# uni-medical/UniMedVL

Measured on AMD Instinct MI355X. Metric: VQA greedy decode tokens/s, UniMedVL-14B (BAGEL-7B-MoT dims), batch 8 x 448x448 per GPU, higher is better.
Workload: dtype bf16; 1 GPU; configs[1]: UniMedVL-14B bf16 VQA greedy decode, batch=8 448x448, 1xMI355X; batch_per_gpu=8, image=448x448, parallelism=dp1, decode=hipGraph

## Files before the change

### unimedvl_amd/csrc/gemm_skinny.h

```cpp
#pragma once
#include "common.h"
#include "../../include/unimedvl_hip.h"
#include "gemm_epilogue.h"
#include "gemm_internal.h"
#include "quant.h"

#define SK_WAVES 8
#define SK_XMAX 16

template <int NT_>
struct SkBf16 {
    static constexpr int NT = NT_, KH = 1;
    static constexpr bool HALVES = false;
    struct Unit { bf16x8 w[NT]; };
    int TH, tile_elems;
    bool rowlane;
    const bf16_t* wbase[NT];
    __device__ __forceinline__ SkBf16(const umv_gemm_args& a, int KT, int NTT, int, int nt0, int lane) {
        const int r = lane & 15, g = lane >> 4;
        TH = a.tile_rows > 0 ? a.tile_rows : 16;
        tile_elems = 4 * TH * 8;
        rowlane = r < TH;
#pragma unroll
        for (int t = 0; t < NT; ++t) {
            const bool tv = (nt0 + t) < NTT;
            wbase[t] = a.wp + ((int64_t)(tv ? nt0 + t : 0) * KT) * tile_elems + (g * TH + (rowlane ? r : 0)) * 8;
        }
    }
    __device__ __forceinline__ void load(Unit& b, int kt, bool ok) const {
#pragma unroll
        for (int t = 0; t < NT; ++t)
            b.w[t] = (ok && rowlane) ? __builtin_nontemporal_load(reinterpret_cast<const bf16x8*>(wbase[t] + (int64_t)kt * tile_elems)) : zero_frag();
    }
    __device__ __forceinline__ void frags(const Unit& b, bf16x8 (&wf)[KH][NT]) const {
#pragma unroll
        for (int t = 0; t < NT; ++t) wf[0][t] = b.w[t];
    }
};

template <int NT_>
struct SkE4m3 {
    static constexpr int NT = NT_, KH = 2, TH = 16;
    static constexpr bool HALVES = false;
    struct Unit { u32x4 w[NT]; };
    const uint8_t* wbase[NT];
    float wscale[NT];
    __device__ __forceinline__ SkE4m3(const umv_gemm_args& a, int KT8, int NTT, int, int nt0, int lane) {
        const uint8_t* wq = reinterpret_cast<const uint8_t*>(a.wp);
#pragma unroll
        for (int t = 0; t < NT; ++t) {
            const bool tv = (nt0 + t) < NTT;
            const int nt = tv ? nt0 + t : 0;
            wbase[t] = wq + ((int64_t)nt * KT8 * 64 + lane) * 16;
            wscale[t] = a.w_scale[nt * 16 + (lane & 15)];
        }
    }
    __device__ __forceinline__ void load(Unit& b, int kt, bool ok) const {
#pragma unroll
        for (int t = 0; t < NT; ++t)
            b.w[t] = ok ? __builtin_nontemporal_load(reinterpret_cast<const u32x4*>(wbase[t] + (int64_t)kt * 1024)) : (u32x4){0u, 0u, 0u, 0u};
    }
    __device__ __forceinline__ void frags(const Unit& b, bf16x8 (&wf)[KH][NT]) const {
#pragma unroll
        for (int t = 0; t < NT; ++t) cvt_fp8x16(b.w[t], wscale[t], wf[0][t], wf[1][t]);
    }
};

template <int NP>
struct SkMxfp4 {
    static constexpr int NT = 2 * NP, KH = 2, TH = 16;
    static constexpr bool HALVES = false;
    struct Unit { u32x4 w[NP]; uint32_t s[NP]; };
    const uint8_t* wbase[NP];
    const uint8_t* sbase[NP];
    __device__ __forceinline__ SkMxfp4(const umv_gemm_args& a, int KT8, int, int NPT, int, int lane) {
        const uint8_t* img = reinterpret_cast<const uint8_t*>(a.wp);
        const uint8_t* scales = img + (int64_t)NPT * KT8 * 1024;
        const int p0 = blockIdx.x * NP;
#pragma unroll
        for (int i = 0; i < NP; ++i) {
            const int p = (p0 + i) < NPT ? p0 + i : 0;
            wbase[i] = img + ((int64_t)p * KT8 * 64 + lane) * 16;
            sbase[i] = scales + ((int64_t)p * KT8 * 16 + (lane & 15)) * 4;
        }
    }
    __device__ __forceinline__ void load(Unit& b, int kt, bool ok) const {
#pragma unroll
        for (int i = 0; i < NP; ++i) {
            b.w[i] = ok ? __builtin_nontemporal_load(reinterpret_cast<const u32x4*>(wbase[i] + (int64_t)kt * 1024)) : (u32x4){0u, 0u, 0u, 0u};
            b.s[i] = ok ? *reinterpret_cast<const uint32_t*>(sbase[i] + (int64_t)kt * 64) : 0x7F7F7F7Fu;
        }
    }
    __device__ __forceinline__ void frags(const Unit& b, bf16x8 (&wf)[KH][NT]) const {
#pragma unroll
        for (int i = 0; i < NP; ++i) {
            const uint32_t s = b.s[i];
            wf[0][2 * i] = cvt_fp4x8(b.w[i].x, e8m0_scale(s & 0xFFu));
            wf[1][2 * i] = cvt_fp4x8(b.w[i].y, e8m0_scale((s >> 8) & 0xFFu));
            wf[0][2 * i + 1] = cvt_fp4x8(b.w[i].z, e8m0_scale((s >> 16) & 0xFFu));
            wf[1][2 * i + 1] = cvt_fp4x8(b.w[i].w, e8m0_scale(s >> 24));
        }
    }
};

typedef __attribute__((ext_vector_type(2))) unsigned short umv_u16x2;
__device__ __forceinline__ uint32_t z13_pk_mad(uint32_t q, uint32_t mul, uint32_t add) {
    const umv_u16x2 r = __builtin_bit_cast(umv_u16x2, q) * __builtin_bit_cast(umv_u16x2, mul) + __builtin_bit_cast(umv_u16x2, add);
    return __builtin_bit_cast(uint32_t, r);
}
__device__ __forceinline__ uint32_t z13_pk_shr8(uint32_t q) {
    const umv_u16x2 r = __builtin_bit_cast(umv_u16x2, q) >> (umv_u16x2){8, 8};
    return __builtin_bit_cast(uint32_t, r);
}
template <int E>
__device__ __forceinline__ bf16x8 z13_frag(uint32_t sm0, uint32_t sm1, uint32_t n, uint32_t t, uint32_t mul, uint32_t base7, uint32_t emask) {
    constexpr int EA = 2 * E, EB = 2 * E + 1;
    const uint32_t ta = EA < 4 ? t << (4 - EA) : t >> (EA - 4), tb = EB < 4 ? t << (4 - EB) : t >> (EB - 4);
    const uint32_t qa = (ta & 0x10101010u) | (n & 0x0F0F0F0Fu), qb = (tb & 0x10101010u) | ((n >> 4) & 0x0F0F0F0Fu);
    const uint32_t e[4] = {z13_pk_mad(qa, mul, base7), z13_pk_mad(z13_pk_shr8(qa), mul, base7), z13_pk_mad(qb, mul, base7),
                           z13_pk_mad(z13_pk_shr8(qb), mul, base7)};
    const uint32_t p[4] = {__builtin_amdgcn_perm(sm0, sm0, 0x01010000u), __builtin_amdgcn_perm(sm0, sm0, 0x03030202u),
                           __builtin_amdgcn_perm(sm1, sm1, 0x01010000u), __builtin_amdgcn_perm(sm1, sm1, 0x03030202u)};
    u32x4 o;
    o.x = (e[0] & emask) | (p[0] & ~emask);
    o.y = (e[1] & emask) | (p[1] & ~emask);
    o.z = (e[2] & emask) | (p[2] & ~emask);
    o.w = (e[3] & emask) | (p[3] & ~emask);
    return __builtin_bit_cast(bf16x8, o);
}

#define Z13_RECORD 3328
__host__ __device__ __forceinline__ int64_t z13_head_bytes(int NPT) { return ((int64_t)NPT * 16 + 255) / 256 * 256; }

template <int NP>
struct SkZ13 {
    static constexpr int NT = 2 * NP, KH = 2, TH = 16;
    static constexpr bool HALVES = true;
    struct Unit { u32x4 sm[NP][2]; u32x4 n[NP]; uint32_t t[NP]; };
    const uint8_t* rec[NP];
    uint32_t base7[NP];
    uint32_t lane16, lane4;
    __device__ __forceinline__ SkZ13(const umv_gemm_args& a, int KT8, int, int NPT, int, int lane) {
        const uint8_t* img = reinterpret_cast<const uint8_t*>(a.wp);
        const int p0 = blockIdx.x * NP;
#pragma unroll
        for (int i = 0; i < NP; ++i) {
            const int p = (p0 + i) < NPT ? p0 + i : 0;
            rec[i] = img + z13_head_bytes(NPT) + (int64_t)p * KT8 * Z13_RECORD;
            const uint32_t b = reinterpret_cast<const uint32_t*>(img)[4 * p + 2] & 0xFFu;
            base7[i] = (b << 7) * 0x10001u;
        }
        lane16 = (uint32_t)lane * 16u;
        lane4 = 3072u + (uint32_t)lane * 4u;
    }
    __device__ __forceinline__ void load(Unit& b, int kt, bool ok) const {
        const int ktu = __builtin_amdgcn_readfirstlane(kt);
#pragma unroll
        for (int i = 0; i < NP; ++i) {
            const uint8_t* r = rec[i] + (int64_t)ktu * Z13_RECORD;
            const u32x4 z = {0u, 0u, 0u, 0u};
            b.sm[i][0] = ok ? __builtin_nontemporal_load(reinterpret_cast<const u32x4*>(r + lane16)) : z;
            b.sm[i][1] = ok ? __builtin_nontemporal_load(reinterpret_cast<const u32x4*>(r + 1024 + lane16)) : z;
            b.n[i] = ok ? __builtin_nontemporal_load(reinterpret_cast<const u32x4*>(r + 2048 + lane16)) : z;
            b.t[i] = ok ? __builtin_nontemporal_load(reinterpret_cast<const uint32_t*>(r + lane4)) : 0u;
        }
    }
    __device__ __forceinline__ void frags(const Unit& b, bf16x8 (&wf)[KH][NT], bool in0, bool in1) const {
        const bool v0 = __builtin_amdgcn_readfirstlane((int)in0) != 0, v1 = __builtin_amdgcn_readfirstlane((int)in1) != 0;
#pragma unroll
        for (int i = 0; i < NP; ++i) {
            const uint32_t mul0 = v0 ? 0xFF80FF80u : 0u, mul1 = v1 ? 0xFF80FF80u : 0u;
            const uint32_t b0 = v0 ? base7[i] : 0u, b1 = v1 ? base7[i] : 0u;
            const uint32_t m0 = v0 ? 0x7F807F80u : 0xFFFFFFFFu, m1 = v1 ? 0x7F807F80u : 0xFFFFFFFFu;
            wf[0][2 * i] = z13_frag<0>(b.sm[i][0].x, b.sm[i][0].y, b.n[i].x, b.t[i], mul0, b0, m0);
            wf[1][2 * i] = z13_frag<1>(b.sm[i][0].z, b.sm[i][0].w, b.n[i].y, b.t[i], mul1, b1, m1);
            wf[0][2 * i + 1] = z13_frag<2>(b.sm[i][1].x, b.sm[i][1].y, b.n[i].z, b.t[i], mul0, b0, m0);
            wf[1][2 * i + 1] = z13_frag<3>(b.sm[i][1].z, b.sm[i][1].w, b.n[i].w, b.t[i], mul1, b1, m1);
        }
    }
};

template <int NW, int NT, int MB>
__device__ __forceinline__ void skinny16_reduce_epilogue(const umv_gemm_args& a, float* red, const f32x4 (&acc)[NT][MB], int tid,
                                                         int lane, int wave, int nt0, int NTT, int nsplit, int TH) {
    constexpr int E4 = NT * MB;
#pragma unroll
    for (int t = 0; t < NT; ++t)
#pragma unroll
        for (int mb = 0; mb < MB; ++mb) reinterpret_cast<f32x4*>(red)[(wave * E4 + t * MB + mb) * 64 + lane] = acc[t][mb];
    __syncthreads();
    EpiCtx e{a.bias, a.residual, a.ldr, a.out, a.ldo, a.N, a.epilogue};
    if (nsplit > 1) {
        e.out = reinterpret_cast<float*>(a.out) + (int64_t)blockIdx.y * a.split_stride;
        e.flags = UMV_EPI_OUT_F32;
    }
    if (a.epilogue & UMV_EPI_SWIGLU) {
        for (int idx = tid; idx < (NT / 2) * MB * 64; idx += NW * 64) {
            int l = idx & 63;
            int f = idx >> 6;
            int pair = f / MB, mb = f % MB;
            f32x4 sg = {0, 0, 0, 0}, su = {0, 0, 0, 0};
#pragma unroll
            for (int w = 0; w < NW; ++w) {
                sg += reinterpret_cast<f32x4*>(red)[(w * E4 + (2 * pair) * MB + mb) * 64 + l];
                su += reinterpret_cast<f32x4*>(red)[(w * E4 + (2 * pair + 1) * MB + mb) * 64 + l];
            }
            int m = mb * 16 + (l & 15);
            int ntile = nt0 + 2 * pair;
            if (m < a.M && ntile < NTT) {
                int64_t orow = a.row_idx ? (int64_t)a.row_idx[m] : (int64_t)m;
                int c0 = (ntile >> 1) * 16 + (l >> 4) * 4;
                float gg[4] = {sg.x, sg.y, sg.z, sg.w}, uu[4] = {su.x, su.y, su.z, su.w};
                epi_swiglu4(e, orow, c0, a.N / 2, gg, uu);
            }
        }
    } else {
        for (int idx = tid; idx < E4 * 64; idx += NW * 64) {
            int l = idx & 63;
            int f = idx >> 6;
            int t = f / MB, mb = f % MB;
            f32x4 s = {0, 0, 0, 0};
#pragma unroll
            for (int w = 0; w < NW; ++w) s += reinterpret_cast<f32x4*>(red)[(w * E4 + f) * 64 + l];
            int m = mb * 16 + (l & 15);
            int n0 = (nt0 + t) * TH + (l >> 4) * 4;
            int nend = min(a.N, (nt0 + t) * TH + TH);
            const bool valid = m < a.M && n0 < nend;
            float fin[4] = {0.f, 0.f, 0.f, 0.f};
            if (valid) {
                int64_t orow = a.row_idx ? (int64_t)a.row_idx[m] : (int64_t)m;
                EpiCtx et = e;
                et.N = nend;
                epi_store4(et, orow, n0, s.x, s.y, s.z, s.w, fin);
            }
            if (a.argmax_partial && nt0 + t < NTT)
                epi_argmax_tile(a.argmax_partial, NTT, m, nt0 + t, l, valid, n0, nend, fin, a.sample_temperature, a.sample_seed, a.sample_step);
        }
    }
}

template <class F, int MB, int U, int XL>
struct SkBuf {
    typename F::Unit w[U];
    bf16x8 x[U][F::KH][MB];
    u32x4 xp[XL ? U * F::KH / 2 : 1][XL == 1 ? 1 : (XL ? 2 * MB : 1)];
};

template <class F, int MB, int U, bool DB, int NORM, int XL>
__device__ __forceinline__ void gemm_skinny_body(const umv_gemm_args& a, int KT, int NTT, int NPT) {
    constexpr int NT = F::NT, KH = F::KH;
    extern __shared__ __attribute__((aligned(16))) float red[];
    const int tid = threadIdx.x;
    const int lane = tid & 63, wave = tid >> 6;
    const int r = lane & 15, g = lane >> 4;
    const int nt0 = blockIdx.x * NT;

    const bf16_t* xrow[MB];
    bool xvalid[MB];
#pragma unroll
    for (int mb = 0; mb < MB; ++mb) {
        int m = mb * 16 + r;
        xvalid[mb] = m < a.M;
        int64_t row = xvalid[mb] ? (a.row_idx ? (int64_t)a.row_idx[m] : (int64_t)m) : 0;
        xrow[mb] = a.x + row * a.ldx;
    }
    f32x4 acc[NT][MB];
#pragma unroll
    for (int t = 0; t < NT; ++t)
#pragma unroll
        for (int mb = 0; mb < MB; ++mb) acc[t][mb] = (f32x4){0.f, 0.f, 0.f, 0.f};

    const int nsplit = a.k_splits > 1 ? a.k_splits : 1;
    constexpr int SG = F::HALVES ? KH : 1;
    const int KTG = KT * SG;
    const int kts = (KTG + nsplit - 1) / nsplit;
    const int ks0 = (int)blockIdx.y * kts, ks1 = min(KTG, ks0 + kts);
    const int kt_per = (max(0, ks1 - ks0) + SK_WAVES - 1) / SK_WAVES;
    const int g_begin = ks0 + wave * kt_per;
    const int g_end = min(ks1, g_begin + kt_per);
    const int kt_begin = g_begin / SG;
    const int kt_end = g_end > g_begin ? (g_end + SG - 1) / SG : kt_begin;
    constexpr int UPL = 2 / KH;
    const int kt_lo = XL != 0 ? (kt_begin & -UPL) : kt_begin;
    const int nk = max(0, kt_end - kt_lo);
    const int nchunks = (nk + U - 1) / U;
    const F f(a, KT, NTT, NPT, nt0, lane);
    static_assert(!XL || ((U * KH) % 2 == 0 && NORM == 0), "full-line x staging: whole lines per chunk, no fused norm");
    static_assert(!F::HALVES || NORM == 0, "half-unit slices: no fused norm");
    static_assert(XL != 1 || MB == 1, "one-piece staging serves one 16-row tile of at most 8 valid rows");
    constexpr int XLN = U * KH / 2, XLP = XL == 1 ? 1 : 2 * MB;
    const int xchunk = (lane & 7) ^ ((lane >> 3) & 7);
    const bf16_t* xprow[XL ? XLP : 1];
    bool xpvalid[XL ? XLP : 1];
    if constexpr (XL != 0) {
#pragma unroll
        for (int q = 0; q < XLP; ++q) {
            const int m = q * 8 + (lane >> 3);
            xpvalid[q] = m < a.M;
            const int64_t row = xpvalid[q] ? (a.row_idx ? (int64_t)a.row_idx[m] : (int64_t)m) : 0;
            xprow[q] = a.x + row * a.ldx + xchunk * 8;
        }
    }
    char* xstage = reinterpret_cast<char*>(red) + wave * (XLN * XLP * 1024);
    auto load_chunk = [&](int c, SkBuf<F, MB, U, XL>& b) {
        if constexpr (XL != 0) {
#pragma unroll
            for (int ln = 0; ln < XLN; ++ln) {
                const int kt = kt_lo + c * U + ln * UPL;
                const int k = kt * (32 * KH) + xchunk * 8;
#pragma unroll
                for (int q = 0; q < XLP; ++q)
                    b.xp[ln][q] = (kt < kt_end && xpvalid[q] && k < a.K) ? *reinterpret_cast<const u32x4*>(xprow[q] + (int64_t)kt * (32 * KH))
                                                                         : (u32x4){0u, 0u, 0u, 0u};
            }
        }
#pragma unroll
        for (int u = 0; u < U; ++u) {
            const int kt = kt_lo + c * U + u;
            const bool ok = kt >= kt_begin && kt < kt_end;
            f.load(b.w[u], kt, ok);
            if (!NORM && XL == 0) {
#pragma unroll
                for (int h = 0; h < KH; ++h) {
                    const int k = kt * (32 * KH) + h * 32 + g * 8;
#pragma unroll
                    for (int mb = 0; mb < MB; ++mb) b.x[u][h][mb] = (ok && xvalid[mb] && k < a.K) ? ldg_frag(xrow[mb] + k) : zero_frag();
                }
            }
        }
    };
    SkBuf<F, MB, U, XL> b0, b1;
    if (nchunks > 0) load_chunk(0, b0);

    constexpr int MP = NORM ? NORM : 8;
    bf16_t* xl = reinterpret_cast<bf16_t*>(red + SK_WAVES * NT * MB * 4 * 64 + SK_WAVES * 16);
    if constexpr (NORM != 0) {
        static_assert(!NORM || MB == 1, "fused RMSNorm supports M <= 16");
        float* part = red + SK_WAVES * NT * MB * 4 * 64;
        const int rr = tid & (MP - 1);
        constexpr int sh = MP == 8 ? 3 : 4;
        constexpr int XS = MP;
        const int nslots = KT * 4 * MP;
        const bool rowok = rr < a.M;
        const bf16_t* xr = a.x + (rowok ? (a.row_idx ? (int64_t)a.row_idx[rr] : (int64_t)rr) : 0) * a.ldx;
        {
            bf16x8 xv[XS];
#pragma unroll
            for (int i = 0; i < XS; ++i) {
                const int sidx = tid + i * SK_WAVES * 64;
                const int k = (sidx >> (sh + 2)) * 32 + ((sidx >> sh) & 3) * 8;
                xv[i] = (sidx < nslots && k < a.K && rowok) ? ldg_frag(xr + k) : zero_frag();
            }
            float ss = 0.f;
#pragma unroll
            for (int i = 0; i < XS; ++i) {
#pragma unroll
                for (int j = 0; j < 8; ++j) {
                    float fv = bf2f((bf16_t)xv[i][j]);
                    ss += fv * fv;
                }
                const int sidx = tid + i * SK_WAVES * 64;
                if (sidx < nslots) *reinterpret_cast<bf16x8*>(xl + (int64_t)sidx * 8) = xv[i];
            }
            if (MP == 8) ss += __shfl_xor(ss, 8, 64);
            ss += __shfl_xor(ss, 16, 64);
            ss += __shfl_xor(ss, 32, 64);
            if (lane < MP) part[wave * 16 + lane] = ss;
        }
        bf16x8 wv[XS];
#pragma unroll
        for (int i = 0; i < XS; ++i) {
            const int sidx = tid + i * SK_WAVES * 64;
            const int k = (sidx >> (sh + 2)) * 32 + ((sidx >> sh) & 3) * 8;
            wv[i] = (sidx < nslots && k < a.K) ? ldg_frag(a.norm_w + k) : zero_frag();
        }
        __syncthreads();
        float tot = 0.f;
#pragma unroll
        for (int w = 0; w < SK_WAVES; ++w) tot += part[w * 16 + rr];
        const float rstd = rsqrt_ieee(tot / (float)a.K + a.norm_eps);
#pragma unroll
        for (int i = 0; i < XS; ++i) {
            const int sidx = tid + i * SK_WAVES * 64;
            if (sidx < nslots) {
                bf16x8 v = *reinterpret_cast<const bf16x8*>(xl + (int64_t)sidx * 8), o;
#pragma unroll
                for (int j = 0; j < 8; ++j) o[j] = (short)f2bf(bf2f((bf16_t)wv[i][j]) * rbf(bf2f((bf16_t)v[j]) * rstd));
                *reinterpret_cast<bf16x8*>(xl + (int64_t)sidx * 8) = o;
            }
        }
        __syncthreads();
    }
    auto consume = [&](SkBuf<F, MB, U, XL>& b, int c) {
        if constexpr (NORM != 0) {
#pragma unroll
            for (int u = 0; u < U; ++u) {
                const int kt = min(kt_begin + c * U + u, KT - 1);
                bf16x8 xf = *reinterpret_cast<const bf16x8*>(xl + ((int64_t)(kt * 4 + g) * MP + (r & (MP - 1))) * 8);
                bf16x8 wf[KH][NT];
                f.frags(b.w[u], wf);
#pragma unroll
                for (int t = 0; t < NT; ++t) acc[t][0] = mfma16(wf[0][t], xf, acc[t][0]);
            }
        } else {
            if constexpr (XL != 0) {
#pragma unroll
                for (int ln = 0; ln < XLN; ++ln)
#pragma unroll
                    for (int q = 0; q < XLP; ++q) *reinterpret_cast<u32x4*>(xstage + (ln * XLP + q) * 1024 + lane * 16) = b.xp[ln][q];
                const int rr = XL == 1 ? (r & 7) : r;
#pragma unroll
                for (int u = 0; u < U; ++u)
#pragma unroll
                    for (int h = 0; h < KH; ++h)
#pragma unroll
                        for (int mb = 0; mb < MB; ++mb) {
                            const int j = u * KH + h;
                            b.x[u][h][mb] = *reinterpret_cast<const bf16x8*>(xstage + (j >> 1) * (XLP * 1024) + (mb * 16 + rr) * 128 +
                                                                             ((((j & 1) * 4 + g) ^ (rr & 7)) << 4));
                        }
            }
#pragma unroll
            for (int u = 0; u < U; ++u) {
                bf16x8 wf[KH][NT];
                if constexpr (F::HALVES) {
                    const int g0 = (kt_lo + c * U + u) * SG;
                    f.frags(b.w[u], wf, g0 >= g_begin && g0 < g_end, g0 + 1 >= g_begin && g0 + 1 < g_end);
                } else {
                    f.frags(b.w[u], wf);
                }
#pragma unroll
                for (int h = 0; h < KH; ++h)
#pragma unroll
                    for (int t = 0; t < NT; ++t)
#pragma unroll
                        for (int mb = 0; mb < MB; ++mb) acc[t][mb] = mfma16(wf[h][t], b.x[u][h][mb], acc[t][mb]);
            }
        }
    };
    for (int c = 0; c < nchunks; c += 2) {
        if (DB && c + 1 < nchunks) load_chunk(c + 1, b1);
        consume(b0, c);
        if (c + 1 < nchunks) {
            if (!DB) load_chunk(c + 1, b1);
            if (c + 2 < nchunks && DB) load_chunk(c + 2, b0);
            consume(b1, c + 1);
            if (c + 2 < nchunks && !DB) load_chunk(c + 2, b0);
        }
    }
    if constexpr (XL != 0) __syncthreads();
    skinny16_reduce_epilogue<SK_WAVES, NT, MB>(a, red, acc, tid, lane, wave, nt0, NTT, nsplit, f.TH);
}

static int skinny_xl() {
    static const int v = umv_env_int("UMV_SKINNY_XL", 2);
    return v;
}

template <int MB, int NT, int U, int KH, int NORM, class Kernel, class... Args>
static int launch_skinny_body(Kernel kernel, const umv_gemm_args& a, int KT, int NTT, hipStream_t s, Args... args) {
    size_t lds = (size_t)SK_WAVES * NT * MB * 4 * 64 * sizeof(float);
    if (NORM) lds += SK_WAVES * 16 * sizeof(float) + (size_t)KT * 4 * NORM * 16;
    auto go = [&](auto XLV) {
        constexpr int XL = decltype(XLV)::value;
        const void* fn = reinterpret_cast<const void*>(kernel(XLV));
        const size_t xl = (size_t)SK_WAVES * (U * KH / 2) * (XL == 1 ? 1 : 2 * MB) * 1024;
        const size_t bytes = XL != 0 && xl > lds ? xl : lds;
        static bool attr_set[UMV_MAX_DEVICES] = {};
        if (bytes > 64 * 1024 && umv_first_on_device(attr_set)) (void)hipFuncSetAttribute(fn, hipFuncAttributeMaxDynamicSharedMemorySize, (int)bytes);
        umv_gemm_args ka = a;
        void* argv[] = {&ka, &args...};
        (void)hipLaunchKernel(fn, dim3((NTT + NT - 1) / NT, a.k_splits > 1 ? a.k_splits : 1), dim3(SK_WAVES * 64), argv, bytes, s);
        UMV_LAUNCH_CHECK();
        return UMV_OK;
    };
    if constexpr (NORM == 0 && (U * KH) % 2 == 0) {
        const int mode = skinny_xl();
        if (mode && (mode > 1 || a.M > 8) && (a.ldx % 64) == 0 && ((uintptr_t)a.x % 128) == 0) {
            if constexpr (MB == 1) {
                if (a.M <= 8) return go(std::integral_constant<int, 1>{});
            }
            return go(std::integral_constant<int, 2>{});
        }
    }
    return go(std::integral_constant<int, 0>{});
}
```

### unimedvl_amd/csrc/gemm_z13.hip

```cpp
#include "common.h"
#include "../../include/unimedvl_hip.h"
#include "gemm_skinny.h"

template <int MB, int NP, int U, int XL = 0>
__global__ __launch_bounds__(SK_WAVES * 64) void gemm_skinny13_kernel(umv_gemm_args a, const uint8_t* z13, int KT8, int NTT, int NPT) {
    const int KT = 2 * KT8, nsplit = a.k_splits > 1 ? a.k_splits : 1;
    const int kts = (KT + nsplit - 1) / nsplit;
    const int ks0 = (int)blockIdx.y * kts, ks1 = min(KT, ks0 + kts);
    uint64_t any = 0;
    if (ks1 > ks0) {
        const int b0 = ks0 >> 4, b1 = (ks1 + 15) >> 4;
        const uint64_t range = (b1 - b0 >= 64 ? ~0ull : ((1ull << (b1 - b0)) - 1ull)) << b0;
        const uint64_t* flags = reinterpret_cast<const uint64_t*>(z13);
#pragma unroll
        for (int i = 0; i < NP; ++i) {
            const int p = (int)blockIdx.x * NP + i;
            if (p < NPT) any |= flags[2 * p] & range;
        }
    }
    if (any != 0) {
        gemm_skinny_body<SkBf16<2 * NP>, MB, 2 * U, true, 0, XL>(a, KT, NTT, 0);
    } else {
        a.wp = reinterpret_cast<const uint16_t*>(z13);
        gemm_skinny_body<SkZ13<NP>, MB, U, true, 0, XL>(a, KT8, NTT, NPT);
    }
}

template <int MB, int NP, int U>
static int launch_skinny13(const umv_gemm_args& a, const uint8_t* z13, int KT8, int NTT, int NPT, hipStream_t s) {
    return launch_skinny_body<MB, 2 * NP, U, 2, 0>([](auto XL) { return &gemm_skinny13_kernel<MB, NP, U, decltype(XL)::value>; }, a, KT8,
                                                   NTT, s, z13, KT8, NTT, NPT);
}

extern "C" int umv_gemm_z13w(const umv_gemm_args* ap, const void* z13, umv_stream_t stream) {
    UMV_CHECK(ap != nullptr, UMV_ERR_ARG, "gemm_z13w: null args");
    umv_gemm_args a = *ap;
    UMV_CHECK(a.x && a.wp && a.out && z13, UMV_ERR_ARG, "gemm_z13w: null pointer (x, wp = the bf16 image, out and z13 are required)");
    UMV_CHECK(!a.w_scale, UMV_ERR_ARG, "gemm_z13w: w_scale must be NULL");
    if (const int rc = umv_gemm_check_args(a, "gemm_z13w", 32)) return rc;
    UMV_CHECK((a.K % 64) == 0 && a.K <= 32768, UMV_ERR_UNSUPPORTED, "gemm_z13w: K (%d) must be a multiple of 64 and <= 32768", a.K);
    UMV_CHECK(a.M <= 64, UMV_ERR_UNSUPPORTED, "gemm_z13w: the 13-bit image is the decode (M <= 64) layout; use umv_gemm_bf16 for M=%d", a.M);
    UMV_CHECK(!a.norm_w && (a.tile_rows == 0 || a.tile_rows == 16), UMV_ERR_UNSUPPORTED, "gemm_z13w: no fused norm / th-row tiles");
    UMV_CHECK(a.k_splits <= 1 || (!(a.epilogue & UMV_EPI_SWIGLU) && a.split_stride > 0 && a.k_splits <= 64), UMV_ERR_UNSUPPORTED,
              "gemm_z13w: split-K (k_splits=%d) needs no SwiGLU, split_stride > 0, k_splits <= 64", a.k_splits);
    UMV_CHECK(!a.argmax_partial || (a.k_splits <= 1 && !a.row_idx && !(a.epilogue & (UMV_EPI_SWIGLU | UMV_EPI_OUT_F32))), UMV_ERR_UNSUPPORTED,
              "gemm_z13w: argmax_partial needs bf16 out, no SwiGLU / split-K / row_idx");
    UMV_CHECK(a.sample_temperature >= 0.f && (a.sample_temperature == 0.f || a.argmax_partial), UMV_ERR_ARG,
              "gemm_z13w: sample_temperature (%g) is a mode of the argmax_partial epilogue and must be >= 0", (double)a.sample_temperature);
    UMV_CHECK(((uintptr_t)z13 % 256) == 0, UMV_ERR_ARG, "gemm_z13w: the 13-bit image must be 256-byte aligned");
    if (a.M == 0) return UMV_OK;
    hipStream_t s = (hipStream_t)stream;
    const uint8_t* z = reinterpret_cast<const uint8_t*>(z13);
    const int KT8 = a.K / 64, NTT = (a.N + 15) / 16, NPT = (NTT + 1) / 2;
    if (a.k_splits > 1) {
        if (a.M <= 16) return launch_skinny13<1, 2, 1>(a, z, KT8, NTT, NPT, s);
        if (a.M <= 32) return launch_skinny13<2, 2, 1>(a, z, KT8, NTT, NPT, s);
        return launch_skinny13<4, 1, 1>(a, z, KT8, NTT, NPT, s);
    }
    const bool two = (a.epilogue & UMV_EPI_SWIGLU) || NTT >= 1024;
    if (a.M <= 16) return launch_skinny13<1, 1, 2>(a, z, KT8, NTT, NPT, s);
    if (a.M <= 32) return two ? launch_skinny13<2, 2, 1>(a, z, KT8, NTT, NPT, s) : launch_skinny13<2, 1, 2>(a, z, KT8, NTT, NPT, s);
    if (two && !a.argmax_partial && a.K >= 1024) return umv_gemm_bf16(&a, stream);
    return launch_skinny13<4, 1, 1>(a, z, KT8, NTT, NPT, s);
}
```

Measured before the change: 2720 tokens/s.

## Add ring-buffered prefetch pipeline to 13-bit skinny GEMM and overlap flag check

The 13-bit decode GEMM for M<=16 now uses a three-deep ring of load buffers with unrolled steady-state stages, replacing the previous double-buffered loop with U=2. The per-block exception-flag check and base exponent read move into the Z13 body. They now come from a header vector loaded in the constructor, and the check runs after the first chunk's loads are already issued, so the flag lookup no longer serialises ahead of the weight stream. If any row is flagged, the body returns false and the kernel falls back to the bf16 path, which now uses a separately chosen unroll. The deeper ring raises register pressure, and fallback blocks issue some wasted Z13 loads.

```diff
diff --git a/unimedvl_amd/csrc/gemm_skinny.h b/unimedvl_amd/csrc/gemm_skinny.h
--- a/unimedvl_amd/csrc/gemm_skinny.h
+++ b/unimedvl_amd/csrc/gemm_skinny.h
@@ -1,4 +1,5 @@
 #pragma once
+#include <utility>
 #include "common.h"
 #include "../../include/unimedvl_hip.h"
 #include "gemm_epilogue.h"
@@ -10,7 +11,7 @@
 
 template <int NT_>
 struct SkBf16 {
-    static constexpr int NT = NT_, KH = 1;
+    static constexpr int NT = NT_, KH = 1, RING = 0;
     static constexpr bool HALVES = false;
     struct Unit { bf16x8 w[NT]; };
     int TH, tile_elems;
@@ -40,7 +41,7 @@
 
 template <int NT_>
 struct SkE4m3 {
-    static constexpr int NT = NT_, KH = 2, TH = 16;
+    static constexpr int NT = NT_, KH = 2, TH = 16, RING = 0;
     static constexpr bool HALVES = false;
     struct Unit { u32x4 w[NT]; };
     const uint8_t* wbase[NT];
@@ -68,7 +69,7 @@
 
 template <int NP>
 struct SkMxfp4 {
-    static constexpr int NT = 2 * NP, KH = 2, TH = 16;
+    static constexpr int NT = 2 * NP, KH = 2, TH = 16, RING = 0;
     static constexpr bool HALVES = false;
     struct Unit { u32x4 w[NP]; uint32_t s[NP]; };
     const uint8_t* wbase[NP];
@@ -132,26 +133,42 @@
 #define Z13_RECORD 3328
 __host__ __device__ __forceinline__ int64_t z13_head_bytes(int NPT) { return ((int64_t)NPT * 16 + 255) / 256 * 256; }
 
-template <int NP>
+template <int NP, int R>
 struct SkZ13 {
-    static constexpr int NT = 2 * NP, KH = 2, TH = 16;
+    static constexpr int NT = 2 * NP, KH = 2, TH = 16, RING = R;
     static constexpr bool HALVES = true;
     struct Unit { u32x4 sm[NP][2]; u32x4 n[NP]; uint32_t t[NP]; };
     const uint8_t* rec[NP];
+    u32x4 head[NP];
+    int npairs;
     uint32_t base7[NP];
     uint32_t lane16, lane4;
     __device__ __forceinline__ SkZ13(const umv_gemm_args& a, int KT8, int, int NPT, int, int lane) {
         const uint8_t* img = reinterpret_cast<const uint8_t*>(a.wp);
         const int p0 = blockIdx.x * NP;
+        npairs = NPT - p0;
 #pragma unroll
         for (int i = 0; i < NP; ++i) {
             const int p = (p0 + i) < NPT ? p0 + i : 0;
             rec[i] = img + z13_head_bytes(NPT) + (int64_t)p * KT8 * Z13_RECORD;
-            const uint32_t b = reinterpret_cast<const uint32_t*>(img)[4 * p + 2] & 0xFFu;
-            base7[i] = (b << 7) * 0x10001u;
+            head[i] = *reinterpret_cast<const u32x4*>(img + (int64_t)p * 16);
         }
         lane16 = (uint32_t)lane * 16u;
         lane4 = 3072u + (uint32_t)lane * 4u;
+    }
+    __device__ __forceinline__ bool flagged(int g0, int g1) const {
+        if (g1 <= g0) return false;
+        const int b0 = g0 >> 4, b1 = (g1 + 15) >> 4;
+        const uint64_t range = (b1 - b0 >= 64 ? ~0ull : ((1ull << (b1 - b0)) - 1ull)) << b0;
+        uint64_t any = 0;
+#pragma unroll
+        for (int i = 0; i < NP; ++i)
+            if (i < npairs) any |= ((uint64_t)head[i].y << 32 | head[i].x) & range;
+        return any != 0;
+    }
+    __device__ __forceinline__ void resolve() {
+#pragma unroll
+        for (int i = 0; i < NP; ++i) base7[i] = ((head[i].z & 0xFFu) << 7) * 0x10001u;
     }
     __device__ __forceinline__ void load(Unit& b, int kt, bool ok) const {
         const int ktu = __builtin_amdgcn_readfirstlane(kt);
@@ -246,14 +263,18 @@
     u32x4 xp[XL ? U * F::KH / 2 : 1][XL == 1 ? 1 : (XL ? 2 * MB : 1)];
 };
 
+template <class Fn, int... S>
+__device__ __forceinline__ void sk_each(Fn&& fn, std::integer_sequence<int, S...>) { (fn(std::integral_constant<int, S>{}), ...); }
+
 template <class F, int MB, int U, bool DB, int NORM, int XL>
-__device__ __forceinline__ void gemm_skinny_body(const umv_gemm_args& a, int KT, int NTT, int NPT) {
+__device__ __forceinline__ bool gemm_skinny_body(const umv_gemm_args& a, int KT, int NTT, int NPT) {
     constexpr int NT = F::NT, KH = F::KH;
     extern __shared__ __attribute__((aligned(16))) float red[];
     const int tid = threadIdx.x;
-    const int lane = tid & 63, wave = tid >> 6;
+    const int lane = tid & 63, wave = F::RING ? __builtin_amdgcn_readfirstlane(tid >> 6) : tid >> 6;
     const int r = lane & 15, g = lane >> 4;
     const int nt0 = blockIdx.x * NT;
+    const int64_t row_none = F::RING && a.row_idx ? (int64_t)a.row_idx[0] : 0;
 
     const bf16_t* xrow[MB];
     bool xvalid[MB];
@@ -261,7 +282,7 @@
     for (int mb = 0; mb < MB; ++mb) {
         int m = mb * 16 + r;
         xvalid[mb] = m < a.M;
-        int64_t row = xvalid[mb] ? (a.row_idx ? (int64_t)a.row_idx[m] : (int64_t)m) : 0;
+        int64_t row = xvalid[mb] ? (a.row_idx ? (int64_t)a.row_idx[m] : (int64_t)m) : row_none;
         xrow[mb] = a.x + row * a.ldx;
     }
     f32x4 acc[NT][MB];
@@ -284,7 +305,7 @@
     const int kt_lo = XL != 0 ? (kt_begin & -UPL) : kt_begin;
     const int nk = max(0, kt_end - kt_lo);
     const int nchunks = (nk + U - 1) / U;
-    const F f(a, KT, NTT, NPT, nt0, lane);
+    F f(a, KT, NTT, NPT, nt0, lane);
     static_assert(!XL || ((U * KH) % 2 == 0 && NORM == 0), "full-line x staging: whole lines per chunk, no fused norm");
     static_assert(!F::HALVES || NORM == 0, "half-unit slices: no fused norm");
     static_assert(XL != 1 || MB == 1, "one-piece staging serves one 16-row tile of at most 8 valid rows");
@@ -297,7 +318,7 @@
         for (int q = 0; q < XLP; ++q) {
             const int m = q * 8 + (lane >> 3);
             xpvalid[q] = m < a.M;
-            const int64_t row = xpvalid[q] ? (a.row_idx ? (int64_t)a.row_idx[m] : (int64_t)m) : 0;
+            const int64_t row = xpvalid[q] ? (a.row_idx ? (int64_t)a.row_idx[m] : (int64_t)m) : row_none;
             xprow[q] = a.x + row * a.ldx + xchunk * 8;
         }
     }
@@ -329,8 +350,37 @@
             }
         }
     };
+    auto load_ring = [&](int c, SkBuf<F, MB, U, XL>& b) {
+        static_assert(!F::RING || (KH == 2 && NORM == 0), "the ring loads whole 64-k lines");
+        if constexpr (XL != 0) {
+#pragma unroll
+            for (int ln = 0; ln < XLN; ++ln) {
+                const int kt = min(kt_lo + c * U + ln, kt_end - 1);
+#pragma unroll
+                for (int q = 0; q < XLP; ++q) b.xp[ln][q] = *reinterpret_cast<const u32x4*>(xprow[q] + (int64_t)kt * 64);
+            }
+        }
+#pragma unroll
+        for (int u = 0; u < U; ++u) {
+            const int kt = min(kt_lo + c * U + u, kt_end - 1);
+            f.load(b.w[u], kt, true);
+            if constexpr (XL == 0) {
+#pragma unroll
+                for (int h = 0; h < KH; ++h)
+#pragma unroll
+                    for (int mb = 0; mb < MB; ++mb) b.x[u][h][mb] = ldg_frag(xrow[mb] + kt * 64 + h * 32 + g * 8);
+            }
+        }
+    };
     SkBuf<F, MB, U, XL> b0, b1;
-    if (nchunks > 0) load_chunk(0, b0);
+    if constexpr (F::RING == 0) {
+        if (nchunks > 0) load_chunk(0, b0);
+        if constexpr (F::HALVES) {
+            __builtin_amdgcn_sched_barrier(0);
+            if (f.flagged(ks0, ks1)) return false;
+            f.resolve();
+        }
+    }
 
     constexpr int MP = NORM ? NORM : 8;
     bf16_t* xl = reinterpret_cast<bf16_t*>(red + SK_WAVES * NT * MB * 4 * 64 + SK_WAVES * 16);
@@ -438,18 +488,51 @@
             }
         }
     };
-    for (int c = 0; c < nchunks; c += 2) {
-        if (DB && c + 1 < nchunks) load_chunk(c + 1, b1);
-        consume(b0, c);
-        if (c + 1 < nchunks) {
-            if (!DB) load_chunk(c + 1, b1);
-            if (c + 2 < nchunks && DB) load_chunk(c + 2, b0);
-            consume(b1, c + 1);
-            if (c + 2 < nchunks && !DB) load_chunk(c + 2, b0);
+    if constexpr (F::RING != 0) {
+        constexpr int R = F::RING;
+        SkBuf<F, MB, U, XL> ring[R];
+        if (nchunks > 0) load_ring(0, ring[0]);
+        __builtin_amdgcn_sched_barrier(0);
+        if (f.flagged(ks0, ks1)) return false;
+        f.resolve();
+        if (nchunks >= R - 1) {
+            sk_each([&](auto D) { load_ring(D.value + 1, ring[D.value + 1]); }, std::make_integer_sequence<int, R - 2>{});
+            int c = 0;
+            auto steady = [&](auto S) {
+                constexpr int s = decltype(S)::value;
+                load_ring(c + R - 1, ring[(s + R - 1) % R]);
+                __builtin_amdgcn_sched_barrier(0);
+                consume(ring[s], c);
+                ++c;
+            };
+            const int steps = nchunks - (R - 1);
+            for (int turn = steps / R; turn > 0; --turn) sk_each(steady, std::make_integer_sequence<int, R>{});
+            const int left = steps % R;
+            sk_each([&](auto L) {
+                if (left == L.value) {
+                    sk_each(steady, std::make_integer_sequence<int, L.value>{});
+                    sk_each([&](auto D) { consume(ring[(L.value + D.value) % R], c + D.value); }, std::make_integer_sequence<int, R - 1>{});
+                }
+            }, std::make_integer_sequence<int, R>{});
+        } else {
+            sk_each([&](auto D) { if (D.value + 1 < nchunks) load_ring(D.value + 1, ring[D.value + 1]); }, std::make_integer_sequence<int, (R > 2 ? R - 3 : 0)>{});
+            sk_each([&](auto D) { if (D.value < nchunks) consume(ring[D.value], D.value); }, std::make_integer_sequence<int, (R > 2 ? R - 2 : 0)>{});
+        }
+    } else {
+        for (int c = 0; c < nchunks; c += 2) {
+            if (DB && c + 1 < nchunks) load_chunk(c + 1, b1);
+            consume(b0, c);
+            if (c + 1 < nchunks) {
+                if (!DB) load_chunk(c + 1, b1);
+                if (c + 2 < nchunks && DB) load_chunk(c + 2, b0);
+                consume(b1, c + 1);
+                if (c + 2 < nchunks && !DB) load_chunk(c + 2, b0);
+            }
         }
     }
     if constexpr (XL != 0) __syncthreads();
     skinny16_reduce_epilogue<SK_WAVES, NT, MB>(a, red, acc, tid, lane, wave, nt0, NTT, nsplit, f.TH);
+    return true;
 }
 
 static int skinny_xl() {
diff --git a/unimedvl_amd/csrc/gemm_z13.hip b/unimedvl_amd/csrc/gemm_z13.hip
--- a/unimedvl_amd/csrc/gemm_z13.hip
+++ b/unimedvl_amd/csrc/gemm_z13.hip
@@ -2,34 +2,19 @@
 #include "../../include/unimedvl_hip.h"
 #include "gemm_skinny.h"
 
-template <int MB, int NP, int U, int XL = 0>
+template <int MB, int NP, int U, int R, int UB, int XL = 0>
 __global__ __launch_bounds__(SK_WAVES * 64) void gemm_skinny13_kernel(umv_gemm_args a, const uint8_t* z13, int KT8, int NTT, int NPT) {
-    const int KT = 2 * KT8, nsplit = a.k_splits > 1 ? a.k_splits : 1;
-    const int kts = (KT + nsplit - 1) / nsplit;
-    const int ks0 = (int)blockIdx.y * kts, ks1 = min(KT, ks0 + kts);
-    uint64_t any = 0;
-    if (ks1 > ks0) {
-        const int b0 = ks0 >> 4, b1 = (ks1 + 15) >> 4;
-        const uint64_t range = (b1 - b0 >= 64 ? ~0ull : ((1ull << (b1 - b0)) - 1ull)) << b0;
-        const uint64_t* flags = reinterpret_cast<const uint64_t*>(z13);
-#pragma unroll
-        for (int i = 0; i < NP; ++i) {
-            const int p = (int)blockIdx.x * NP + i;
-            if (p < NPT) any |= flags[2 * p] & range;
-        }
-    }
-    if (any != 0) {
-        gemm_skinny_body<SkBf16<2 * NP>, MB, 2 * U, true, 0, XL>(a, KT, NTT, 0);
-    } else {
-        a.wp = reinterpret_cast<const uint16_t*>(z13);
-        gemm_skinny_body<SkZ13<NP>, MB, U, true, 0, XL>(a, KT8, NTT, NPT);
-    }
+    umv_gemm_args az = a;
+    az.wp = reinterpret_cast<const uint16_t*>(z13);
+    if (!gemm_skinny_body<SkZ13<NP, R>, MB, U, true, 0, XL>(az, KT8, NTT, NPT))
+        gemm_skinny_body<SkBf16<2 * NP>, MB, UB, true, 0, XL>(a, 2 * KT8, NTT, 0);
 }
 
-template <int MB, int NP, int U>
+template <int MB, int NP, int U, int R, int UB>
 static int launch_skinny13(const umv_gemm_args& a, const uint8_t* z13, int KT8, int NTT, int NPT, hipStream_t s) {
-    return launch_skinny_body<MB, 2 * NP, U, 2, 0>([](auto XL) { return &gemm_skinny13_kernel<MB, NP, U, decltype(XL)::value>; }, a, KT8,
-                                                   NTT, s, z13, KT8, NTT, NPT);
+    constexpr int LINES = U > UB / 2 ? U : UB / 2;
+    return launch_skinny_body<MB, 2 * NP, LINES, 2, 0>([](auto XL) { return &gemm_skinny13_kernel<MB, NP, U, R, UB, decltype(XL)::value>; },
+                                                       a, KT8, NTT, s, z13, KT8, NTT, NPT);
 }
 
 extern "C" int umv_gemm_z13w(const umv_gemm_args* ap, const void* z13, umv_stream_t stream) {
@@ -53,13 +38,13 @@
     const uint8_t* z = reinterpret_cast<const uint8_t*>(z13);
     const int KT8 = a.K / 64, NTT = (a.N + 15) / 16, NPT = (NTT + 1) / 2;
     if (a.k_splits > 1) {
-        if (a.M <= 16) return launch_skinny13<1, 2, 1>(a, z, KT8, NTT, NPT, s);
-        if (a.M <= 32) return launch_skinny13<2, 2, 1>(a, z, KT8, NTT, NPT, s);
-        return launch_skinny13<4, 1, 1>(a, z, KT8, NTT, NPT, s);
+        if (a.M <= 16) return launch_skinny13<1, 2, 1, 0, 2>(a, z, KT8, NTT, NPT, s);
+        if (a.M <= 32) return launch_skinny13<2, 2, 1, 0, 2>(a, z, KT8, NTT, NPT, s);
+        return launch_skinny13<4, 1, 1, 0, 2>(a, z, KT8, NTT, NPT, s);
     }
     const bool two = (a.epilogue & UMV_EPI_SWIGLU) || NTT >= 1024;
-    if (a.M <= 16) return launch_skinny13<1, 1, 2>(a, z, KT8, NTT, NPT, s);
-    if (a.M <= 32) return two ? launch_skinny13<2, 2, 1>(a, z, KT8, NTT, NPT, s) : launch_skinny13<2, 1, 2>(a, z, KT8, NTT, NPT, s);
+    if (a.M <= 16) return launch_skinny13<1, 1, 1, 3, 4>(a, z, KT8, NTT, NPT, s);
+    if (a.M <= 32) return two ? launch_skinny13<2, 2, 1, 0, 2>(a, z, KT8, NTT, NPT, s) : launch_skinny13<2, 1, 2, 0, 4>(a, z, KT8, NTT, NPT, s);
     if (two && !a.argmax_partial && a.K >= 1024) return umv_gemm_bf16(&a, stream);
-    return launch_skinny13<4, 1, 1>(a, z, KT8, NTT, NPT, s);
+    return launch_skinny13<4, 1, 1, 0, 2>(a, z, KT8, NTT, NPT, s);
 }
```

Result: no change. 2742 tokens/s (median of 6 runs) (+0.8%).
